# Corleone-Huang/DynamicVectorQuantization

Hardware: AMD Instinct MI355X
Metric: images encoded/sec (VQ hot path: gate + routing + VQ assign), 256x256 inputs, K=1024 (higher is better)
Workload: dtype f32; 1 GPU; BASELINE configs[2]: dqvae-entropy-dual-r05, B=256 per GPU, 32x32x256 latents, K=1024, entropy gate + dual routing + VectorQuantize2 assign as one op (quant_conv not in the path); global_batch=256, assign_mode=filter, spinup_steps=100, streams=3, repeats=1, full=False, parallelism=single GPU: no exchange runs, world=1, distinct_devices=1

## Files before the change

dynamicvectorquantization_amd/csrc/dvq_pass1.h:

```cpp
#pragma once
#include "dvq_filter.h"
#include <type_traits>

#define DVQ_LOAD_Z(p) __builtin_nontemporal_load(p)
#define DVQ_STORE_ZQ(p, v) __builtin_nontemporal_store((v), (p))
#define DVQ_BUF_LOAD(rsrc, voff, soff, AUX) __builtin_bit_cast(float, __builtin_amdgcn_raw_buffer_load_b32((rsrc), (voff), (soff), (AUX)))
#define DVQ_BUF_STORE(v, rsrc, voff, soff) __builtin_amdgcn_raw_buffer_store_b32(__builtin_bit_cast(unsigned, (float)(v)), (rsrc), (voff), (soff), 2)
#define DVQ_BUF_LOAD16(XT, rsrc, voff, soff, AUX) dvq_widen_bits<XT>(__builtin_amdgcn_raw_buffer_load_b16((rsrc), (voff), (soff), (AUX)))
#define DVQ_BUF_STORE16(XT, v, rsrc, voff, soff) __builtin_amdgcn_raw_buffer_store_b16(dvq_narrow_bits<XT>(v), (rsrc), (voff), (soff), 2)
#define DVQ_LOAD_SEL(p) (*(p))

#ifdef DVQ_TUNING
#ifdef __HIP_DEVICE_COMPILE__
#define DVQ_TUNING_PTR __device__
#else
#define DVQ_TUNING_PTR static __device__
#endif
DVQ_TUNING_PTR float *g_dvq_tokdbg __asm__("g_dvq_tokdbg") = nullptr;
DVQ_TUNING_PTR unsigned long long *g_dvq_stamps __asm__("g_dvq_stamps") = nullptr;
#define DVQ_STAMP(i) do { if (SPLIT && g_dvq_stamps != nullptr && threadIdx.x == 0) g_dvq_stamps[(size_t)blockIdx.x * 8 + (i)] = wall_clock64(); } while (0)
static inline int dvq_tuning_set_unit(void *stamps, void *tokdbg)
{
    int rc = (int)hipMemcpyToSymbol(HIP_SYMBOL(g_dvq_stamps), &stamps, sizeof(void *));
    if (rc) return rc;
// ... 78 lines not shown
        if constexpr (RES) {
#pragma unroll
            for (int k = 0; k < SEED_TILES / 2 / NW; ++k) {
                const int pair = wave * (SEED_TILES / 2 / NW) + k;
                const int t0 = (2 * pair < T) ? 2 * pair : T - 1;
                const unsigned voff = (unsigned)c * 4u + ((t0 + 1 < T) ? (unsigned)h * (unsigned)TILE_STRIDE : 0u);
                glds4(img + (size_t)t0 * TILE_STRIDE + IMG_BYTES + voff, enraw + pair * 64);
            }
        }
    };
    const int tile_id = SPLIT ? (int)(blockIdx.x / (unsigned)ksplit) : xcd_swizzle(blockIdx.x, gridDim.x);
    const int pre = (SEL == 2) ? ((rv.G == 2) ? 2 : 1) : 3;

    const int n_raw = (tile_id * NW + wave) * 32 + c;
    const int n = (n_raw < N) ? n_raw : -1;
    auto token_base = [&](int HW, int h) -> size_t {
        const long nn = (n >= 0) ? n : N - 1;
        if constexpr (FLAT) return (size_t)nn * D + 8 * h;
        const long bimg = nn / HW;
        const int hw = (int)(nn - bimg * HW);
        return ((size_t)bimg * D + 8 * h) * HW + hw;
    };
    auto wave_base = [&](const float *p0, int hw, int hh) -> __amdgpu_buffer_rsrc_t {
        const size_t tb = token_base(hw, hh);
        const size_t tb0 = ((size_t)(unsigned)__builtin_amdgcn_readfirstlane((int)(tb >> 32)) << 32) |
                           (size_t)(unsigned)__builtin_amdgcn_readfirstlane((int)(tb & 0xFFFFFFFFu));
        if constexpr (XT != 0) return __builtin_amdgcn_make_buffer_rsrc((void *)((const char *)p0 + tb0 * ZB), 0, -1, 0x00020000);
        else return __builtin_amdgcn_make_buffer_rsrc((void *)(p0 + tb0), 0, -1, 0x00020000);
    };
    auto lane_off = [&](int hw, int hh) -> unsigned {
        const size_t tb = token_base(hw, hh);
        const size_t tb0 = ((size_t)(unsigned)__builtin_amdgcn_readfirstlane((int)(tb >> 32)) << 32) |
                           (size_t)(unsigned)__builtin_amdgcn_readfirstlane((int)(tb & 0xFFFFFFFFu));
        return (unsigned)(tb - tb0) * (XT ? 2u : 4u);
    };
    float zf[S16][8];
    float sel_mask = 1.0f;
    int sel_g = 0;
    unsigned stg_a = 0, stg_b = 0;
    auto conv_prologue = [&](const float *zp, size_t st) __attribute__((always_inline)) {
        constexpr int QIMG = S16 * 1024;
        constexpr int QTILE = 2 * QIMG + 256;
        float *bias_l = enraw;
        float xr[3][8];
        const float *xp = zp;
        auto issue_w = [&](int k, int q) __attribute__((always_inline)) {
            const int i = 4 * wave + q;
            glds16(cv.wimg + (size_t)(i >> 1) * QTILE + (i & 1) * QIMG + k * 1024 + lane * 16,
                   lds + (k & 3) * IMG_BYTES + i * 1024);
        };
        auto issue_x = [&](int k, int j) __attribute__((always_inline)) {
            asm volatile("global_load_dword %0, %1, off nt" : "=v"(xr[k % 3][j]) : "v"(xp) : "memory");
            xp += (j == 7) ? 9 * st : st;
        };
        auto issue_group = [&](int k) __attribute__((always_inline)) {
#pragma unroll
            for (int q = 0; q < 4; ++q) issue_w(k, q);
#pragma unroll
            for (int j = 0; j < 8; ++j) issue_x(k, j);
        };
        glds4(cv.bias + wave * 64 + lane, bias_l + wave * 64);
        issue_group(0);
        issue_group(1);
        issue_group(2);
        f32x16 acc[8];
#pragma unroll
        for (int t8 = 0; t8 < 8; ++t8)
#pragma unroll
            for (int r = 0; r < 16; ++r) acc[t8][r] = 0.0f;
        int ea = 100;
        float sa = ldexpf(1.0f, 100);
        f16x8 xh, xl;
        auto take_group = [&](int g) __attribute__((always_inline)) {
            if (g <= S16 - 3) asm volatile("s_waitcnt vmcnt(24)" ::: "memory");
            else if (g == S16 - 2) asm volatile("s_waitcnt vmcnt(12)" ::: "memory");
            else asm volatile("s_waitcnt vmcnt(0)" ::: "memory");
            float xv[8];
#pragma unroll
            for (int j = 0; j < 8; ++j) { asm volatile("" : "+v"(xr[g % 3][j])); xv[j] = xr[g % 3][j]; }
            float m = 0.0f;
#pragma unroll
            for (int j = 0; j < 8; ++j) m = vmax_abs(m, xv[j]);
            m = fmaxf(m, __shfl_xor(m, 32));
            const bool grow = (m > 0.0f) && (m < __builtin_inff()) && (m * sa >= 32768.0f);
            if (__builtin_amdgcn_ballot_w64(grow) != 0ull) {
                int e;
                (void)frexpf(grow ? m : 1.0f, &e);
                int en = 14 - e;
                en = en > 100 ? 100 : (en < -100 ? -100 : en);
                en = grow ? en : ea;
                if (g > 0) {
                    const float f = ldexpf(1.0f, en - ea);
#pragma unroll
                    for (int t8 = 0; t8 < 8; ++t8)
#pragma unroll
                        for (int r = 0; r < 16; ++r) acc[t8][r] *= f;
                }
                ea = en;
                sa = ldexpf(1.0f, ea);
            }
            u32x4 ph, pl;
#pragma unroll
            for (int j2 = 0; j2 < 4; ++j2) {
                const float v0 = xv[2 * j2] * sa, v1 = xv[2 * j2 + 1] * sa;
                const f32x2 vv = {v0, v1};
                const f16x2 hh = __builtin_convertvector(vv, f16x2);
                const f32x2 rr = {v0 - (float)hh[0], v1 - (float)hh[1]};
                const f16x2 ll = __builtin_convertvector(rr, f16x2);
                ph[j2] = __builtin_bit_cast(unsigned, hh);
                pl[j2] = __builtin_bit_cast(unsigned, ll);
            }
            xh = __builtin_bit_cast(f16x8, ph);
            xl = __builtin_bit_cast(f16x8, pl);
        };
        take_group(0);
#pragma unroll
        for (int s = 0; s < S16; ++s) {
            __builtin_amdgcn_s_barrier();
            asm volatile("" ::: "memory");
            const f16x8 bh = xh, bl = xl;
            const unsigned wa = (unsigned)(size_t)(const __attribute__((address_space(3))) char *)(lds + (s & 3) * IMG_BYTES) + lane * 16;
            f16x8 wf[3];
#define CV_OFF(Q) ((((Q) & 1) ? ((Q) - 1) : ((Q) + 1)) * 1024)
#define CV_RD(Q) asm volatile("ds_read_b128 %0, %1 offset:%c2" : "=v"(wf[(Q) % 3]) : "v"(wa), "i"(CV_OFF(Q)))
#define CV_WAIT(N, Q) asm volatile("s_waitcnt lgkmcnt(" #N ")" : "+v"(wf[(Q) % 3]) :: "memory")
            CV_RD(0); CV_RD(1); CV_RD(2);
            __builtin_amdgcn_sched_barrier(0);
#define CV_TILE(T8, W0, W1)                                                                                              \
            CV_WAIT(W0, 2 * (T8));                                                                                        \
            __builtin_amdgcn_sched_barrier(0);                                                                            \
            acc[T8] = __builtin_amdgcn_mfma_f32_32x32x16_f16(wf[(2 * (T8)) % 3], bh, acc[T8], 0, 0, 0);    \
            __builtin_amdgcn_sched_barrier(0);                                                                            \
            if (2 * (T8) + 3 < 16) { CV_RD(2 * (T8) + 3 < 16 ? 2 * (T8) + 3 : 0); }                                       \
            CV_WAIT(W1, 2 * (T8) + 1);                                                                                    \
            __builtin_amdgcn_sched_barrier(0);                                                                            \
            acc[T8] = __builtin_amdgcn_mfma_f32_32x32x16_f16(wf[(2 * (T8) + 1) % 3], bl, acc[T8], 0, 0, 0);               \
            acc[T8] = __builtin_amdgcn_mfma_f32_32x32x16_f16(wf[(2 * (T8) + 1) % 3], bh, acc[T8], 0, 0, 0);               \
            __builtin_amdgcn_sched_barrier(0);                                                                            \
            if (2 * (T8) + 4 < 16) { CV_RD(2 * (T8) + 4 < 16 ? 2 * (T8) + 4 : 0); }
#define CV_W(Q) if (s + 3 < S16) { issue_w(s + 3, Q); __builtin_amdgcn_sched_barrier(0); }
#define CV_X(J) if (s + 3 < S16) { issue_x(s + 3, J); issue_x(s + 3, (J) + 1); __builtin_amdgcn_sched_barrier(0); }
            CV_TILE(0, 2, 2) CV_W(0) CV_TILE(1, 2, 2) CV_W(1) CV_TILE(2, 2, 2) CV_W(2) CV_TILE(3, 2, 2) CV_W(3)
            CV_TILE(4, 2, 2) CV_X(0) CV_TILE(5, 2, 2) CV_X(2) CV_TILE(6, 2, 2) CV_X(4) CV_TILE(7, 1, 0) CV_X(6)
#undef CV_W
#undef CV_X
#undef CV_TILE
#undef CV_WAIT
#undef CV_RD
#undef CV_OFF
            __builtin_amdgcn_sched_barrier(0);
            if (s + 1 < S16) take_group(s + 1);
        }
        const float unscale = ldexpf(cv.meta->inv_scale_w, -ea);
#pragma unroll
        for (int s = 0; s < S16; ++s) {
            const f32x4 b0 = *(const f32x4 *)(bias_l + 16 * s + 8 * h), b1v = *(const f32x4 *)(bias_l + 16 * s + 8 * h + 4);
#pragma unroll
            for (int j = 0; j < 8; ++j)
                zf[s][j] = __builtin_fmaf(acc[s >> 1][8 * (s & 1) + j], unscale, (j < 4) ? b0[j & 3] : b1v[j & 3]);
            __builtin_amdgcn_sched_barrier(0);
        }
        if (cv.h_all && n >= 0) {
            float *hp = cv.h_buf + token_base(HW, h);
#pragma unroll
            for (int s = 0; s < S16; ++s)
#pragma unroll
                for (int j = 0; j < 8; ++j) hp[(size_t)(16 * s + j) * HW] = zf[s][j];
        }
        __builtin_amdgcn_s_barrier();
        asm volatile("" ::: "memory");
        issue_seeds();
        for (int t = 0; t < 3; ++t) issue(t);
        __builtin_amdgcn_sched_barrier(0);
    };
    if (SEL != 0) {
        const int nn = (n >= 0) ? n : (int)(N - 1);
        const int b = nn / HW, pos = nn - b * HW;
        const int y = pos / rv.Wout, x = pos - y * rv.Wout;
        const int SC = rv.sub[rv.G - 1];
        const size_t cell = (size_t)b * rv.hc * rv.wc + (y / SC) * rv.wc + x / SC;
        const DvqGateRaw graw = dvq_gate_fetch(rv.gate, rv.gate_mode, rv.G, cell);
        auto by_products = [&](int g) {
            const int rep_g = rv.rep[g];
            sel_mask = 1.0f / (float)(rep_g * rep_g);
            if (n >= 0 && h == 0 && rv.cmask_out != nullptr) {
                rv.cmask_out[n] = sel_mask;
                if (y % SC == 0 && x % SC == 0) {
                    rv.indices_out[cell] = g;
                    if (rv.gate_mode == 2 && rv.gate_out != nullptr) {
                        const float e = graw.f[0];
                        longlong2 gg; gg.x = (e <= rv.thr) ? 1 : 0; gg.y = (e > rv.thr) ? 1 : 0;
                        *(longlong2 *)(rv.gate_out + 2 * cell) = gg;
                    }
                }
            }
            if (!(y % rep_g == 0 && x % rep_g == 0)) sel_mask = -sel_mask;
        };
        if (SEL == 1) {
            const int g = dvq_gate_reduce(graw, rv.gate_mode, rv.G, rv.thr);
            by_products(g);
            int stride_l;
            const float *zp = dvq_dense_source(rv, b, y, x, g, stride_l) + (size_t)8 * h * stride_l;
            const size_t st = (size_t)stride_l;
            if constexpr (CONV) {
                conv_prologue(zp, st);
            } else {
            issue_seeds();
            for (int t = 0; t < pre; ++t) issue(t);
            __builtin_amdgcn_s_setprio(2);
#pragma unroll
            for (int s = 0; s < S16; ++s)
#pragma unroll
                for (int j = 0; j < 8; ++j) zf[s][j] = DVQ_LOAD_SEL(zp + (size_t)(16 * s + j) * st);
            __builtin_amdgcn_s_setprio(0);
            }
        } else {
            issue_seeds();
            for (int t = 0; t < pre; ++t) issue(t);
            const int bw = __builtin_amdgcn_readfirstlane(b);
            const int y0 = __builtin_amdgcn_readfirstlane(y) - wave;
            char *img_a = lds + pre * IMG_BYTES;
            char *img_b = lds + 3 * IMG_BYTES;
            {
                const int ga = rv.G - 2;
                const int plane = rv.hc * rv.sub[ga] * 16;
                const float *src = rv.src[ga] + (size_t)bw * D * plane + (size_t)(y0 >> 1) * 16 + (lane & 7) * 4;
                for (int i = wave; i < D / 8; i += NW)
                    glds16(src + (size_t)(i * 8 + (lane >> 3)) * plane, img_a + i * 1024);
            }
            if (rv.G == 3) {
                const int plane = rv.hc * 8;
                const float *src = rv.src[0] + (size_t)bw * D * plane + (size_t)(y0 >> 2) * 8 + (lane & 1) * 4;
                for (int i = wave; i < D / 32; i += NW)
                    glds16(src + (size_t)(i * 32 + (lane >> 1)) * plane, img_b + i * 1024);
            }
            stg_a = (unsigned)(size_t)(const __attribute__((address_space(3))) char *)img_a +
                    (unsigned)((8 * h) * 128 + (((wave >> 1) * 16 + (c >> 1)) << 2));
            stg_b = (unsigned)(size_t)(const __attribute__((address_space(3))) char *)img_b +
                    (unsigned)((8 * h) * 32 + ((c >> 2) << 2));
            const __amdgpu_buffer_rsrc_t zr = __builtin_amdgcn_make_buffer_rsrc((void *)(rv.src[rv.G - 1] + (size_t)bw * D * HW), 0,
                                                                                -1, 0x00020000);
            const unsigned zo = (unsigned)(8 * h * HW + pos) * 4u;
            __builtin_amdgcn_s_setprio(2);
#pragma unroll
            for (int s = 0; s < S16; ++s)
#pragma unroll
                for (int j = 0; j < 8; ++j) zf[s][j] = DVQ_BUF_LOAD(zr, zo, (16 * s + j) * HW * 4, NT ? 2 : 0);
            __builtin_amdgcn_s_setprio(0);
            asm volatile("s_waitcnt vmcnt(0)" ::: "memory");
            __builtin_amdgcn_s_barrier();
            asm volatile("" ::: "memory");
            sel_g = dvq_gate_reduce(graw, rv.gate_mode, rv.G, rv.thr);
            by_products(sel_g);
        }
    } else if constexpr (CONV) {
        conv_prologue(z + token_base(HW, h), (size_t)HW);
    } else if constexpr (FLAT) {
        char *tr = lds + wave * FLAT_TRW;
        const long n0 = ((long)tile_id * NW + wave) * 32;
        f32x4 tmp[2][FLAT_IPH];
#pragma unroll
        for (int h2 = 0; h2 < 2; ++h2)
#pragma unroll
            for (int i = 0; i < FLAT_IPH; ++i) {
                long tk = n0 + i * FLAT_TPI + lane / FLAT_LPT;
                tk = tk < N ? tk : N - 1;
                const f32x4 *src = (const f32x4 *)(z + (size_t)tk * D + h2 * (D / 2)) + (lane % FLAT_LPT);
                tmp[h2][i] = NT ? __builtin_nontemporal_load(src) : *src;
            }
#pragma unroll
        for (int h2 = 0; h2 < 2; ++h2) {
#pragma unroll
            for (int i = 0; i < FLAT_IPH; ++i)
                *(f32x4 *)(tr + (i * FLAT_TPI + lane / FLAT_LPT) * FLAT_RSH + (lane % FLAT_LPT) * 16) = tmp[h2][i];
#pragma unroll
            for (int sp = 0; sp < S16 / 2; ++sp) {
                const int s = h2 * (S16 / 2) + sp;
                const f32x4 lo = *(const f32x4 *)(tr + c * FLAT_RSH + (16 * sp + 8 * h) * 4);
                const f32x4 hi = *(const f32x4 *)(tr + c * FLAT_RSH + (16 * sp + 8 * h + 4) * 4);
#pragma unroll
                for (int j = 0; j < 4; ++j) { zf[s][j] = lo[j]; zf[s][4 + j] = hi[j]; }
            }
        }
        __syncthreads();
        issue_seeds();
        for (int t = 0; t < pre; ++t) issue(t);
    } else {
        issue_seeds();
        for (int t = 0; t < pre; ++t) issue(t);
        const __amdgpu_buffer_rsrc_t zr = wave_base(z, HW, h);
        const unsigned zo = lane_off(HW, h);
        __builtin_amdgcn_s_setprio(2);
#pragma unroll
        for (int s = 0; s < S16; ++s)
#pragma unroll
            for (int j = 0; j < 8; ++j) {
                if constexpr (XT != 0) zf[s][j] = DVQ_BUF_LOAD16(XT, zr, zo, (16 * s + j) * HW * 2, NT ? 2 : 0);
                else zf[s][j] = DVQ_BUF_LOAD(zr, zo, (16 * s + j) * HW * 4, NT ? 2 : 0);
            }
        __builtin_amdgcn_s_setprio(0);
    }
    f16x8 zb[2][S32];
    float xn, thr2W;
    {
        float pa[2][8];
        float amax = 0.0f, zeta2 = 0.0f;
        f16x8 zprev = {};
#pragma unroll
        for (int s = 0; s < S16; ++s) {
            if (SEL == 2) {
                if (sel_g == rv.G - 2) {
#pragma unroll
                    for (int j = 0; j < 8; ++j)
                        asm volatile("ds_read_b32 %0, %1 offset:%c2" : "+v"(zf[s][j]) : "v"(stg_a), "i"((16 * s + j) * 128));
                    asm volatile("s_waitcnt lgkmcnt(0)" ::: "memory");
                }
                if (rv.G == 3 && sel_g == 0) {
#pragma unroll
                    for (int j = 0; j < 8; ++j)
                        asm volatile("ds_read_b32 %0, %1 offset:%c2" : "+v"(zf[s][j]) : "v"(stg_b), "i"((16 * s + j) * 32));
                    asm volatile("s_waitcnt lgkmcnt(0)" ::: "memory");
                }
#pragma unroll
                for (int j = 0; j < 8; ++j) asm volatile("" : "+v"(zf[s][j]));
            }
            u32x4 packed;
#pragma unroll
            for (int j2 = 0; j2 < 4; ++j2) {
                const float v0 = zf[s][2 * j2], v1 = zf[s][2 * j2 + 1];
                const float q0 = sq_rn(v0), q1 = sq_rn(v1);
                pa[s & 1][2 * j2] = (s < 2) ? q0 : __fadd_rn(pa[s & 1][2 * j2], q0);
                pa[s & 1][2 * j2 + 1] = (s < 2) ? q1 : __fadd_rn(pa[s & 1][2 * j2 + 1], q1);
                amax = vmax_abs(amax, v0);
                amax = vmax_abs(amax, v1);
                f32x2 vv = {v0, v1};
                f16x2 hh = __builtin_convertvector(vv, f16x2);
                packed[j2] = __builtin_bit_cast(unsigned, hh);
                const float r0 = v0 - (float)hh[0], r1 = v1 - (float)hh[1];
                zeta2 = __builtin_fmaf(r0, r0, zeta2);
                zeta2 = __builtin_fmaf(r1, r1, zeta2);
            }
            if constexpr (SEL == 2) {
                asm volatile("" : "+v"(packed), "+v"(zeta2));
                if (sel_mask < 0.0f) packed = u32x4{0u, 0u, 0u, 0u};
            }
            const f16x8 zcur = __builtin_bit_cast(f16x8, packed);
            if (s & 1) {
                const int sp = s >> 1;
                *(f16x8 *)(scr + lane * 16) = zprev;
                *(f16x8 *)(scr + 1024 + lane * 16) = zcur;
#pragma unroll
                for (int t2 = 0; t2 < 2; ++t2) {
                    const int srcl = 16 * t2 + (lane & 15) + 32 * ((lane >> 4) & 1);
                    zb[t2][sp] = *(const f16x8 *)(scr + (lane >> 5) * 1024 + srcl * 16);
                }
            }
            zprev = zcur;
            if constexpr (CONV) __builtin_amdgcn_sched_barrier(0);
        }
        float t8[8];
#pragma unroll
        for (int l = 0; l < 8; ++l) {
            float o0 = __shfl_xor(pa[0][l], 32), o1 = __shfl_xor(pa[1][l], 32);
            float a0 = h == 0 ? pa[0][l] : o0;
            float a1 = h == 0 ? o0 : pa[0][l];
            float a2 = h == 0 ? pa[1][l] : o1;
            float a3 = h == 0 ? o1 : pa[1][l];
            t8[l] = __fadd_rn(__fadd_rn(__fadd_rn(a0, a1), a2), a3);
        }
        xn = t8[0];
#pragma unroll
        for (int l = 1; l < 8; ++l) xn = __fadd_rn(xn, t8[l]);
        amax = fmaxf(amax, __shfl_xor(amax, 32));
        zeta2 += __shfl_xor(zeta2, 32);
        thr2W = FOLD ? dvq_fold_threshold(xn, amax, zeta2, sB, (const DvqFoldMeta *)meta)
                     : dvq_filter_threshold(xn, amax, zeta2, sB, meta);
    }
    if (SEL == 2) {
        __builtin_amdgcn_s_barrier();
        asm volatile("" ::: "memory");
    }
    for (int t = pre; t < 3; ++t) issue(t);
    DVQ_STAMP(1);

    float best, second;
    int code;
    {
        const int q16 = lane >> 4;
        float b1[2] = {-__builtin_inff(), -__builtin_inff()}, b2[2] = {-__builtin_inff(), -__builtin_inff()};
        int bt[2] = {0, 0};
        f32x4 acc16[2][2];
        auto top2 = [&](int tt) {
#pragma unroll
            for (int t2 = 0; t2 < 2; ++t2) {
                const float om = b1[t2];
#pragma unroll
                for (int r = 0; r < 8; r += 2) {
                    const float v0 = acc16[r >> 2][t2][r & 3], v1 = acc16[(r + 1) >> 2][t2][(r + 1) & 3];
                    float g0 = __uint_as_float((__float_as_uint(v0) & 0xFFFFFFF0u) | (unsigned)r);
                    float g1 = __uint_as_float((__float_as_uint(v1) & 0xFFFFFFF0u) | (unsigned)(r + 1));
                    float md = __builtin_amdgcn_fmed3f(b1[t2], g0, g1);
                    b1[t2] = vmax3_raw(b1[t2], g0, g1);
                    b2[t2] = vmax_raw(b2[t2], md);
                }
                bt[t2] = (b1[t2] != om) ? tt : bt[t2];
            }
        };
    for (int t = 0; t < T; ++t) {
            asm volatile("s_waitcnt vmcnt(%0)" ::"n"(PER_TILE) : "memory");
            __builtin_amdgcn_s_barrier();
            asm volatile("" ::: "memory");
            if (S16 != 16) issue(t + 3);
            const unsigned tile_a = (unsigned)(size_t)(const __attribute__((address_space(3))) char *)(
                                        lds + (t & (NBUF - 1)) * IMG_BYTES + lane * 16);
            f16x8 a0, a1, a2, a3;
#define DVQ_RD(dst, S) asm volatile("ds_read_b128 %0, %1 offset:%c2" : "=v"(dst) : "v"(tile_a), "i"((S) * 1024))
            DVQ_RD(a0, 0); DVQ_RD(a1, 1); DVQ_RD(a2, 2); DVQ_RD(a3, 3);
            __builtin_amdgcn_sched_barrier(0);
            if (t > 0) top2(t - 1);
            __builtin_amdgcn_sched_barrier(0);
            {
                const unsigned seed_a = (unsigned)(size_t)(const __attribute__((address_space(3))) char *)(
                                            RES ? enraw + t * 32 + 4 * q16 : enraw + ((t & (NBUF - 1)) * NW + wave) * 64 + 4 * q16);
                f32x4 e0, e1;
                asm volatile("ds_read_b128 %0, %1" : "=v"(e0) : "v"(seed_a));
                asm volatile("ds_read_b128 %0, %1 offset:64" : "=v"(e1) : "v"(seed_a));
                asm volatile("s_waitcnt lgkmcnt(0)" : "+v"(e0), "+v"(e1), "+v"(a0), "+v"(a1), "+v"(a2), "+v"(a3) :: "memory");
                acc16[0][0] = e0; acc16[0][1] = e0; acc16[1][0] = e1; acc16[1][1] = e1;
            }
            __builtin_amdgcn_sched_barrier(0);
#define DVQ_PIECE(Q) if constexpr ((Q) < PER_TILE) { issue_piece(t + 3, Q); }
#define DVQ_MM(src, F, WAIT, NEXT)                                                                             \
            asm volatile("s_waitcnt lgkmcnt(" #WAIT ")" ::: "memory");                                            \
            __builtin_amdgcn_sched_barrier(0);                                                                    \
            acc16[(F) / S32][0] = __builtin_amdgcn_mfma_f32_16x16x32_f16(src, zb[0][(F) % S32], acc16[(F) / S32][0], 0, 0, 0); \
            acc16[(F) / S32][1] = __builtin_amdgcn_mfma_f32_16x16x32_f16(src, zb[1][(F) % S32], acc16[(F) / S32][1], 0, 0, 0); \
            __builtin_amdgcn_sched_barrier(0);                                                                    \
            if ((F) + 4 < S16) { DVQ_RD(src, ((F) + 4 < S16 ? (F) + 4 : 0)); }                                  \
            NEXT
            __builtin_amdgcn_s_setprio(1);
            if (S16 == 16) {
                DVQ_MM(a0, 0, 0, ) DVQ_MM(a1, 1, 1, DVQ_PIECE(0)) DVQ_MM(a2, 2, 2, ) DVQ_MM(a3, 3, 3, )
                DVQ_MM(a0, 4, 3, DVQ_PIECE(1)) DVQ_MM(a1, 5, 3, ) DVQ_MM(a2, 6, 3, ) DVQ_MM(a3, 7, 3, DVQ_PIECE(2))
                DVQ_MM(a0, 8, 3, ) DVQ_MM(a1, 9, 3, ) DVQ_MM(a2, 10, 3, DVQ_PIECE(3)) DVQ_MM(a3, 11, 3, )
                DVQ_MM(a0, 12, 3, ) DVQ_MM(a1, 13, 2, DVQ_PIECE(4)) DVQ_MM(a2, 14, 1, ) DVQ_MM(a3, 15, 0, )
            } else if (S16 == 8) {
                DVQ_MM(a0, 0, 0, ) DVQ_MM(a1, 1, 1, ) DVQ_MM(a2, 2, 2, ) DVQ_MM(a3, 3, 3, )
                DVQ_MM(a0, 4, 3, ) DVQ_MM(a1, 5, 2, ) DVQ_MM(a2, 6, 1, ) DVQ_MM(a3, 7, 0, )
            } else {
                DVQ_MM(a0, 0, 0, ) DVQ_MM(a1, 1, 0, ) DVQ_MM(a2, 2, 0, ) DVQ_MM(a3, 3, 0, )
            }
#undef DVQ_MM
#undef DVQ_RD
#undef DVQ_PIECE
            __builtin_amdgcn_s_setprio(0);
        }
        top2(T - 1);
        asm volatile("s_waitcnt vmcnt(0)" ::: "memory");
        float rb[2], rs[2];
        int rc[2];
#pragma unroll
        for (int t2 = 0; t2 < 2; ++t2) {
            float mb = b1[t2], ms = b2[t2];
            int mt = bt[t2], mq = q16;
#pragma unroll
            for (int off = 16; off <= 32; off <<= 1) {
                const float o1 = __shfl_xor(mb, off), o2 = __shfl_xor(ms, off);
                const int ot = __shfl_xor(mt, off), oq = __shfl_xor(mq, off);
                const bool other_wins = (o1 > mb) || (o1 == mb && ((lane ^ off) < lane));
                ms = fmaxf(other_wins ? mb : o1, fmaxf(ms, o2));
                mb = other_wins ? o1 : mb;
                mt = other_wins ? ot : mt;
                mq = other_wins ? oq : mq;
            }
            const int r = (int)(__float_as_uint(mb) & 15u);
            rb[t2] = mb;
            rs[t2] = ms;
            rc[t2] = (mt + t_lo) * 32 + 16 * (r >> 2) + 4 * mq + (r & 3);
        }
        const int srcl = c & 15;
        const float x0 = __shfl(rb[0], srcl), x1 = __shfl(rb[1], srcl);
        const float y0 = __shfl(rs[0], srcl), y1 = __shfl(rs[1], srcl);
        const int c0 = __shfl(rc[0], srcl), c1 = __shfl(rc[1], srcl);
        best = (c >> 4) ? x1 : x0;
        second = (c >> 4) ? y1 : y0;
        code = (c >> 4) ? c1 : c0;
    }
    DVQ_STAMP(2);
    if constexpr (SEL == 2) {
        const int lane_e = (int)__builtin_amdgcn_mbcnt_hi(~0u, __builtin_amdgcn_mbcnt_lo(~0u, 0u));
        const int c_e = lane_e & 31;
        float am = __builtin_fabsf(sel_mask);
        asm volatile("" : "+v"(am));
        const int rm1 = (am == 1.0f) ? 0 : ((am == 0.25f) ? 1 : 3);
        char *hand = lds + NBUF * IMG_BYTES + NBUF * NW * 64 * 4;
        if (lane_e < 32) {
            const f32x4 mine = {best, second, __int_as_float(code), 0.0f};
            *(f32x4 *)(hand + wave * 2048 + c_e * 16) = mine;
        }
        __syncthreads();
        const f32x4 own = *(const f32x4 *)(hand + (wave - (wave & rm1)) * 2048 + (c_e - (c_e & rm1)) * 16);
        best = own[0];
        second = own[1];
        code = __float_as_int(own[2]);
    }
    if constexpr (SPLIT) {
        typedef __attribute__((address_space(1))) unsigned long long gu64;
        __shared__ int s_last;
        gu64 *mine = (gu64 *)(split + ((size_t)tile_id * ksplit) * 128 + wave * 32 + c);
        if (h == 0) {
            gu64 *e = mine + (size_t)ks * 128 * 2;
            __hip_atomic_store(e, ((unsigned long long)__float_as_uint(second) << 32) | __float_as_uint(best), __ATOMIC_RELAXED, __HIP_MEMORY_SCOPE_AGENT);
            __hip_atomic_store(e + 1, (unsigned long long)(unsigned)code, __ATOMIC_RELAXED, __HIP_MEMORY_SCOPE_AGENT);
        }
        asm volatile("s_waitcnt vmcnt(0)" ::: "memory");
        __syncthreads();
        DVQ_STAMP(3);
        if (tid == 0) {
            const int old = __hip_atomic_fetch_add(&counters[DVQ_SPLIT_TICKET0 + tile_id], 1, __ATOMIC_RELAXED, __HIP_MEMORY_SCOPE_AGENT);
            s_last = (old == ksplit - 1);
            if (old == ksplit - 1)
                __hip_atomic_store(&counters[DVQ_SPLIT_TICKET0 + tile_id], 0, __ATOMIC_RELAXED, __HIP_MEMORY_SCOPE_AGENT);
        }
        __syncthreads();
        DVQ_STAMP(4);
        if (!s_last) return;
        float mb = -__builtin_inff(), ms = -__builtin_inff();
        int mc = 0;
        unsigned long long e0[DVQ_SPLIT_MAX_SLICES], e1[DVQ_SPLIT_MAX_SLICES];
#pragma unroll
        for (int k = 0; k < DVQ_SPLIT_MAX_SLICES; ++k) {
            const int kk = k < ksplit ? k : ksplit - 1;
            e0[k] = __hip_atomic_load(mine + (size_t)kk * 128 * 2, __ATOMIC_RELAXED, __HIP_MEMORY_SCOPE_AGENT);
            e1[k] = __hip_atomic_load(mine + (size_t)kk * 128 * 2 + 1, __ATOMIC_RELAXED, __HIP_MEMORY_SCOPE_AGENT);
        }
#pragma unroll
        for (int k = 0; k < DVQ_SPLIT_MAX_SLICES; ++k) {
            const float eb = __uint_as_float((unsigned)e0[k]), es = __uint_as_float((unsigned)(e0[k] >> 32));
            const bool other_wins = k < ksplit && eb > mb;
            ms = (k < ksplit) ? fmaxf(other_wins ? mb : eb, fmaxf(ms, es)) : ms;
            mc = other_wins ? (int)(unsigned)e1[k] : mc;
            mb = other_wins ? eb : mb;
        }
        best = mb; second = ms; code = mc;
        DVQ_STAMP(5);
    }
    const float thr = best - thr2W;
    const bool final_ok = (best - second) > thr2W;
    const bool valid = n >= 0;
    bool hopeless = !(code < K) || !(thr == thr);
#ifdef DVQ_TUNING
    if (g_dvq_tokdbg != nullptr && valid && h == 0) {
        f32x4 dbg = {best, second, thr2W, (float)code};
        *(f32x4 *)(g_dvq_tokdbg + 4 * (size_t)n) = dbg;
    }
#endif
    const bool undecided = valid && !hopeless && !final_ok;
    const int sel_rep = (SEL == 0 || sel_mask < 0.0f) ? (SEL == 0 ? 1 : 0) : (sel_mask == 1.0f ? 1 : (sel_mask == 0.25f ? 2 : 4));
    const bool queued = undecided && sel_rep > 0;
    const unsigned long long umask = __ballot(queued && h == 0);
    const int shard = (SPLIT ? tile_id * NW + wave : (int)blockIdx.x) & (DVQ_QSHARDS - 1);
    int slot_raw = 0;
    if (umask != 0ull && lane == 0) slot_raw = atomicAdd(&counters[DVQ_QCOUNT0 + shard], (int)__popcll(umask));
    if (valid && hopeless && h == 0) {
        int pos = atomicAdd(&counters[DVQ_C_EXACT], 1);
        exact_list[pos] = n;
    }
    float lsum = 0.0f;
    float m_tok = 1.0f;
    if (valid && !hopeless) {
        if (h == 0) codes[n] = (long long)code;
        m_tok = (SEL != 0) ? __builtin_fabsf(sel_mask) : ((mask != nullptr) ? mask[n] : 1.0f);
        if (zq != nullptr || partials != nullptr) {
            int h_e = h;
            if constexpr (FOLD || (FLAT && SPLIT) || SEL == 2) h_e =(int)(__builtin_amdgcn_mbcnt_hi(~0u, __builtin_amdgcn_mbcnt_lo(~0u, 0u)) >> 5);
            const float *ep = E + (size_t)code * D + 8 * h_e;
            constexpr int SB = SPLIT ? ((S16 < 8) ? S16 : 8) : ((S16 < 2) ? S16 : 2);
            auto finish = [&](auto store_tag) {
                constexpr bool STORE = decltype(store_tag)::value;
                int hw_e = HW;
                asm volatile("" : "+s"(hw_e));
                const __amdgpu_buffer_rsrc_t qr = wave_base(STORE ? zq : (float *)E, hw_e, h_e);
                const unsigned qo = lane_off(hw_e, h_e);
                int hw4 = HW * (XT ? 2 : 4);
                asm volatile("" : "+s"(hw4));
#pragma unroll
                for (int s0 = 0; s0 < S16; s0 += SB) {
                    f32x4 eg[SB][2];
#pragma unroll
                    for (int q = 0; q < SB; ++q) {
                        eg[q][0] = *(const f32x4 *)(ep + 16 * (s0 + q));
                        eg[q][1] = *(const f32x4 *)(ep + 16 * (s0 + q) + 4);
                    }
#pragma unroll
                    for (int q = 0; q < SB; ++q) {
                        const int s = s0 + q;
#pragma unroll
                        for (int j = 0; j < 8; ++j) {
                            float e = eg[q][j >> 2][j & 3];
                            if constexpr (FOLD) {
                                if (STORE) DVQ_BUF_STORE(e, qr, qo, (16 * s + j) * hw4);
                            } else {
                            float diff = __fsub_rn(e, zf[s][j]);
                            if constexpr (XT != 0) {
                                if (STORE) DVQ_BUF_STORE16(XT, __fadd_rn(zf[s][j], diff), qr, qo, (16 * s + j) * hw4);
                            } else
                            if (STORE) DVQ_BUF_STORE(__fadd_rn(zf[s][j], diff), qr, qo, (16 * s + j) * hw4);
                            lsum = __builtin_fmaf(diff, diff, lsum);
                            }
                        }
                    }
                }
            };
            if constexpr (!FLAT) {
                if (zq != nullptr) finish(std::true_type{});
                else finish(std::false_type{});
                lsum *= m_tok;
            }
        }
    }
    if constexpr (FLAT) {
        char *flat_tr = lds + wave * FLAT_TRW;
        const bool store = zq != nullptr;
        if (store) __syncthreads();
        const bool mine = valid && !hopeless && (store || partials != nullptr);
        const unsigned long long okmask = __ballot(valid && !hopeless && h == 0);
        const long n0 = ((long)tile_id * NW + wave) * 32;
        const float *ep = E + (size_t)(mine ? code : 0) * D + 8 * h;
#pragma unroll
        for (int h2 = 0; h2 < 2; ++h2) {
            if (mine) {
                constexpr int SB = (S16 / 2 < 2) ? S16 / 2 : 2;
#pragma unroll
                for (int sp0 = 0; sp0 < S16 / 2; sp0 += SB) {
                    f32x4 eg[SB][2];
#pragma unroll
                    for (int q = 0; q < SB; ++q) {
                        eg[q][0] = *(const f32x4 *)(ep + 16 * (h2 * (S16 / 2) + sp0 + q));
                        eg[q][1] = *(const f32x4 *)(ep + 16 * (h2 * (S16 / 2) + sp0 + q) + 4);
                    }
#pragma unroll
                    for (int q = 0; q < SB; ++q) {
                        const int sp = sp0 + q, s = h2 * (S16 / 2) + sp;
                        f32x4 o[2];
#pragma unroll
                        for (int j = 0; j < 8; ++j) {
                            const float e = eg[q][j >> 2][j & 3];
                            if constexpr (FOLD) {
                                o[j >> 2][j & 3] = e;
                            } else {
                                const float diff = __fsub_rn(e, zf[s][j]);
                                o[j >> 2][j & 3] = __fadd_rn(zf[s][j], diff);
                                lsum = __builtin_fmaf(diff, diff, lsum);
                            }
                        }
                        if (store) {
                            *(f32x4 *)(flat_tr + c * FLAT_RSH + (16 * sp + 8 * h) * 4) = o[0];
                            *(f32x4 *)(flat_tr + c * FLAT_RSH + (16 * sp + 8 * h + 4) * 4) = o[1];
                        }
                    }
                }
            }
            if (store) {
#pragma unroll
                for (int i = 0; i < FLAT_IPH; ++i) {
                    const int tk = i * FLAT_TPI + lane / FLAT_LPT;
                    const f32x4 v = *(const f32x4 *)(flat_tr + tk * FLAT_RSH + (lane % FLAT_LPT) * 16);
                    if ((okmask >> tk) & 1ull)
                        __builtin_nontemporal_store(v, (f32x4 *)(zq + (size_t)(n0 + tk) * D + h2 * (D / 2)) + (lane % FLAT_LPT));
                }
            }
        }
        lsum *= m_tok;
    }
    DVQ_STAMP(6);
    if (umask != 0ull) {
        const int base = __shfl(slot_raw, 0);
        int slot = base + (int)__popcll(umask & ((1ull << c) - 1ull));
        slot = queued ? slot : -1;
        if (queued && slot >= rec_cap) {
            if (h == 0) {
                const int rr = sel_rep > 0 ? sel_rep : 1;
                for (int ry = 0; ry < rr; ++ry)
                    for (int rx = 0; rx < rr; ++rx) {
                        int pos = atomicAdd(&counters[DVQ_C_EXACT], 1);
                        exact_list[pos] = n + ry * rv.Wout + rx;
                    }
            }
            lsum = -(float)(sel_rep * sel_rep - 1) * lsum;
            slot = -1;
        }
        if (slot >= 0) {
            char *rec = records + ((size_t)shard * rec_cap + slot) * rec_bytes(D);
#pragma unroll
            for (int s = 0; s < S16; ++s) {
                f32x4 lo = {zf[s][0], zf[s][1], zf[s][2], zf[s][3]};
                f32x4 hi = {zf[s][4], zf[s][5], zf[s][6], zf[s][7]};
                *(f32x4 *)(rec + (16 * s + 8 * h) * 4) = lo;
                *(f32x4 *)(rec + (16 * s + 8 * h + 4) * 4) = hi;
            }
            if (h == 0) {
                RecMeta rm;
                rm.n = n; rm.xn = xn; rm.thr = thr; rm.m = m_tok; rm.prov = code;
                rm.best = ~0ull; rm.rep = sel_rep > 0 ? sel_rep : 1;
                *(RecMeta *)(rec + (size_t)D * 4) = rm;
            }
        }
    }
    if (partials != nullptr) {
        double dsum = (double)lsum;
#pragma unroll
        for (int off = 32; off > 0; off >>= 1) dsum += __shfl_xor(dsum, off);
        __syncthreads();
        double *red = (double *)lds;
        if (lane == 0) red[wave] = dsum;
        __syncthreads();
        if (tid == 0) partials[SPLIT ? tile_id : (int)blockIdx.x] = (red[0] + red[1]) + (red[2] + red[3]);
    }
    DVQ_STAMP(7);
}

template <int D, int SEL, bool CONV, bool FOLD, bool RES>
__global__ __launch_bounds__(256, 2) void vq_assign_filter_kernel(
    const float *__restrict__ z, const char *__restrict__ img, const DvqF16Meta *__restrict__ meta,
    const float *__restrict__ E, const float *__restrict__ mask,
    int HW, int K, long N, float *__restrict__ zq, long long *__restrict__ codes,
    double *__restrict__ partials, int *__restrict__ counters, int *__restrict__ exact_list,
    char *__restrict__ records, int rec_cap, const DvqRouted rv, const DvqConv cv)
{
    pass1_body<D, SEL, CONV, FOLD, true, RES>(z, img, meta, E, mask, HW, K, N, zq, codes, partials, counters, exact_list, records, rec_cap, rv, cv);
}

template <int D, bool FOLD, bool RES>
__global__ __launch_bounds__(256, 2) void vq_assign_filter_flat_kernel(
    const float *__restrict__ z, const char *__restrict__ img, const DvqF16Meta *__restrict__ meta,
    const float *__restrict__ E, const float *__restrict__ mask,
    int HW, int K, long N, float *__restrict__ zq, long long *__restrict__ codes,
    double *__restrict__ partials, int *__restrict__ counters, int *__restrict__ exact_list,
    char *__restrict__ records, int rec_cap, const DvqRouted rv, const DvqConv cv)
{
    pass1_body<D, 0, false, FOLD, true, RES, true>(z, img, meta, E, mask, HW, K, N, zq, codes, partials, counters, exact_list, records, rec_cap, rv, cv);
}

template <int D, int SEL, bool CONV, bool FOLD, bool FLAT, bool RES>
__global__ __launch_bounds__(256, 2) void vq_assign_filter_split_kernel(
    const float *__restrict__ z, const char *__restrict__ img, const DvqF16Meta *__restrict__ meta,
    const float *__restrict__ E, const float *__restrict__ mask,
    int HW, int K, long N, float *__restrict__ zq, long long *__restrict__ codes,
    double *__restrict__ partials, int *__restrict__ counters, int *__restrict__ exact_list,
    char *__restrict__ records, int rec_cap, const DvqRouted rv, const DvqConv cv, f32x4 *__restrict__ split, int ksplit)
{
    pass1_body<D, SEL, CONV, FOLD, CONV, RES, FLAT, true>(z, img, meta, E, mask, HW, K, N, zq, codes, partials, counters, exact_list, records,
                                                     rec_cap, rv, cv, split, ksplit);
}

template <int D, int SEL, bool FOLD, bool RES>
__global__ __launch_bounds__(256, 2) void vq_assign_filter_cached_kernel(
    const float *__restrict__ z, const char *__restrict__ img, const DvqF16Meta *__restrict__ meta,
    const float *__restrict__ E, const float *__restrict__ mask,
    int HW, int K, long N, float *__restrict__ zq, long long *__restrict__ codes,
    double *__restrict__ partials, int *__restrict__ counters, int *__restrict__ exact_list,
    char *__restrict__ records, int rec_cap, const DvqRouted rv, const DvqConv cv)
{
    pass1_body<D, SEL, false, FOLD, false, RES>(z, img, meta, E, mask, HW, K, N, zq, codes, partials, counters, exact_list, records, rec_cap, rv, cv);
}

template <int D, bool RES, int XT>
__global__ __launch_bounds__(256, 2) void vq_assign_filter_x16_kernel(
    const void *__restrict__ z, const char *__restrict__ img, const DvqF16Meta *__restrict__ meta,
    const float *__restrict__ E, const float *__restrict__ mask,
    int HW, int K, long N, void *__restrict__ zq, long long *__restrict__ codes,
    double *__restrict__ partials, int *__restrict__ counters, int *__restrict__ exact_list,
    char *__restrict__ records, int rec_cap)
{
    static_assert(XT == 1 || XT == 2, "f16 or bf16");
    pass1_body<D, 0, false, false, true, RES, false, false, XT>((const float *)z, img, meta, E, mask, HW, K, N, (float *)zq, codes, partials,
                                                                counters, exact_list, records, rec_cap, DvqRouted{}, DvqConv{});
}

struct FilterWs {
    int *counters, *chunk_sync, *exact_list;
    char *records;
    int cap;
    f32x4 *split;
};

enum class P1Form { plain, cached, flat, split, wide, x16 };
struct P1Plan {
    P1Form form;
// ... 121 lines not shown
```

Baseline: 1.324 million images/s.

## Compact live token columns and skip half the MFMAs when enough are masked

For the dual-routing select path, builds a per-wave permutation that packs active token columns first and masked copy columns last, so the B operand layout places live tokens in the first 16-column group. When at least 16 columns are masked copies, a single-group variant of the distance loop runs, issuing half the MFMAs and top-2 updates. Results are then un-permuted with a popcount-based lane map. This adds an LDS table, extra ballot/popcount logic and a duplicated, wave-uniform-branched loop body that increases code size and register pressure.

```diff
diff --git a/dynamicvectorquantization_amd/csrc/dvq_pass1.h b/dynamicvectorquantization_amd/csrc/dvq_pass1.h
--- a/dynamicvectorquantization_amd/csrc/dvq_pass1.h
+++ b/dynamicvectorquantization_amd/csrc/dvq_pass1.h
@@ -404,6 +404,20 @@
     }
     f16x8 zb[2][S32];
     float xn, thr2W;
+    unsigned copymask = 0u;
+    unsigned perm_off[2] = {0u, 0u};
+    if constexpr (SEL == 2) {
+        copymask = (unsigned)__builtin_amdgcn_ballot_w64(sel_mask < 0.0f && h == 0);
+        const int below = __builtin_popcount(copymask & ((1u << c) - 1u));
+        const int p = (sel_mask < 0.0f) ? 32 - __builtin_popcount(copymask) + below : c - below;
+        unsigned char *tab = (unsigned char *)scr;
+        if (h == 0) tab[p] = (unsigned char)c;
+#pragma unroll
+        for (int t2 = 0; t2 < 2; ++t2) {
+            const unsigned col = tab[16 * t2 + (lane & 15)];
+            perm_off[t2] = (unsigned)(lane >> 5) * 1024u + (col + 32u * ((unsigned)(lane >> 4) & 1u)) * 16u;
+        }
+    }
     {
         float pa[2][8];
         float amax = 0.0f, zeta2 = 0.0f;
@@ -453,8 +467,12 @@
                 *(f16x8 *)(scr + 1024 + lane * 16) = zcur;
 #pragma unroll
                 for (int t2 = 0; t2 < 2; ++t2) {
+                    if constexpr (SEL == 2) {
+                        zb[t2][sp] = *(const f16x8 *)(scr + perm_off[t2]);
+                    } else {
                     const int srcl = 16 * t2 + (lane & 15) + 32 * ((lane >> 4) & 1);
                     zb[t2][sp] = *(const f16x8 *)(scr + (lane >> 5) * 1024 + srcl * 16);
+                    }
                 }
             }
             zprev = zcur;
@@ -491,73 +509,21 @@
         const int q16 = lane >> 4;
         float b1[2] = {-__builtin_inff(), -__builtin_inff()}, b2[2] = {-__builtin_inff(), -__builtin_inff()};
         int bt[2] = {0, 0};
-        f32x4 acc16[2][2];
-        auto top2 = [&](int tt) {
-#pragma unroll
-            for (int t2 = 0; t2 < 2; ++t2) {
-                const float om = b1[t2];
-#pragma unroll
-                for (int r = 0; r < 8; r += 2) {
-                    const float v0 = acc16[r >> 2][t2][r & 3], v1 = acc16[(r + 1) >> 2][t2][(r + 1) & 3];
-                    float g0 = __uint_as_float((__float_as_uint(v0) & 0xFFFFFFF0u) | (unsigned)r);
-                    float g1 = __uint_as_float((__float_as_uint(v1) & 0xFFFFFFF0u) | (unsigned)(r + 1));
-                    float md = __builtin_amdgcn_fmed3f(b1[t2], g0, g1);
-                    b1[t2] = vmax3_raw(b1[t2], g0, g1);
-                    b2[t2] = vmax_raw(b2[t2], md);
-                }
-                bt[t2] = (b1[t2] != om) ? tt : bt[t2];
-            }
-        };
-    for (int t = 0; t < T; ++t) {
-            asm volatile("s_waitcnt vmcnt(%0)" ::"n"(PER_TILE) : "memory");
-            __builtin_amdgcn_s_barrier();
-            asm volatile("" ::: "memory");
-            if (S16 != 16) issue(t + 3);
-            const unsigned tile_a = (unsigned)(size_t)(const __attribute__((address_space(3))) char *)(
-                                        lds + (t & (NBUF - 1)) * IMG_BYTES + lane * 16);
-            f16x8 a0, a1, a2, a3;
-#define DVQ_RD(dst, S) asm volatile("ds_read_b128 %0, %1 offset:%c2" : "=v"(dst) : "v"(tile_a), "i"((S) * 1024))
-            DVQ_RD(a0, 0); DVQ_RD(a1, 1); DVQ_RD(a2, 2); DVQ_RD(a3, 3);
-            __builtin_amdgcn_sched_barrier(0);
-            if (t > 0) top2(t - 1);
-            __builtin_amdgcn_sched_barrier(0);
-            {
-                const unsigned seed_a = (unsigned)(size_t)(const __attribute__((address_space(3))) char *)(
-                                            RES ? enraw + t * 32 + 4 * q16 : enraw + ((t & (NBUF - 1)) * NW + wave) * 64 + 4 * q16);
-                f32x4 e0, e1;
-                asm volatile("ds_read_b128 %0, %1" : "=v"(e0) : "v"(seed_a));
-                asm volatile("ds_read_b128 %0, %1 offset:64" : "=v"(e1) : "v"(seed_a));
-                asm volatile("s_waitcnt lgkmcnt(0)" : "+v"(e0), "+v"(e1), "+v"(a0), "+v"(a1), "+v"(a2), "+v"(a3) :: "memory");
-                acc16[0][0] = e0; acc16[0][1] = e0; acc16[1][0] = e1; acc16[1][1] = e1;
-            }
-            __builtin_amdgcn_sched_barrier(0);
-#define DVQ_PIECE(Q) if constexpr ((Q) < PER_TILE) { issue_piece(t + 3, Q); }
-#define DVQ_MM(src, F, WAIT, NEXT)                                                                             \
-            asm volatile("s_waitcnt lgkmcnt(" #WAIT ")" ::: "memory");                                            \
-            __builtin_amdgcn_sched_barrier(0);                                                                    \
-            acc16[(F) / S32][0] = __builtin_amdgcn_mfma_f32_16x16x32_f16(src, zb[0][(F) % S32], acc16[(F) / S32][0], 0, 0, 0); \
-            acc16[(F) / S32][1] = __builtin_amdgcn_mfma_f32_16x16x32_f16(src, zb[1][(F) % S32], acc16[(F) / S32][1], 0, 0, 0); \
-            __builtin_amdgcn_sched_barrier(0);                                                                    \
-            if ((F) + 4 < S16) { DVQ_RD(src, ((F) + 4 < S16 ? (F) + 4 : 0)); }                                  \
-            NEXT
-            __builtin_amdgcn_s_setprio(1);
-            if (S16 == 16) {
-                DVQ_MM(a0, 0, 0, ) DVQ_MM(a1, 1, 1, DVQ_PIECE(0)) DVQ_MM(a2, 2, 2, ) DVQ_MM(a3, 3, 3, )
-                DVQ_MM(a0, 4, 3, DVQ_PIECE(1)) DVQ_MM(a1, 5, 3, ) DVQ_MM(a2, 6, 3, ) DVQ_MM(a3, 7, 3, DVQ_PIECE(2))
-                DVQ_MM(a0, 8, 3, ) DVQ_MM(a1, 9, 3, ) DVQ_MM(a2, 10, 3, DVQ_PIECE(3)) DVQ_MM(a3, 11, 3, )
-                DVQ_MM(a0, 12, 3, ) DVQ_MM(a1, 13, 2, DVQ_PIECE(4)) DVQ_MM(a2, 14, 1, ) DVQ_MM(a3, 15, 0, )
-            } else if (S16 == 8) {
-                DVQ_MM(a0, 0, 0, ) DVQ_MM(a1, 1, 1, ) DVQ_MM(a2, 2, 2, ) DVQ_MM(a3, 3, 3, )
-                DVQ_MM(a0, 4, 3, ) DVQ_MM(a1, 5, 2, ) DVQ_MM(a2, 6, 1, ) DVQ_MM(a3, 7, 0, )
+        if constexpr (SEL == 2) {
+            if (__builtin_popcount(copymask) >= 16) {
+#define DVQ_NG 1
+#include "pass1_loop.h"
+#undef DVQ_NG
             } else {
-                DVQ_MM(a0, 0, 0, ) DVQ_MM(a1, 1, 0, ) DVQ_MM(a2, 2, 0, ) DVQ_MM(a3, 3, 0, )
-            }
-#undef DVQ_MM
-#undef DVQ_RD
-#undef DVQ_PIECE
-            __builtin_amdgcn_s_setprio(0);
-        }
-        top2(T - 1);
+#define DVQ_NG 2
+#include "pass1_loop.h"
+#undef DVQ_NG
+            }
+        } else {
+#define DVQ_NG 2
+#include "pass1_loop.h"
+#undef DVQ_NG
+        }
         asm volatile("s_waitcnt vmcnt(0)" ::: "memory");
         float rb[2], rs[2];
         int rc[2];
@@ -580,6 +546,20 @@
             rs[t2] = ms;
             rc[t2] = (mt + t_lo) * 32 + 16 * (r >> 2) + 4 * mq + (r & 3);
         }
+        if constexpr (SEL == 2) {
+            unsigned cm = copymask;
+            asm volatile("" : "+s"(cm));
+            const int c_p = (int)__builtin_amdgcn_mbcnt_hi(~0u, __builtin_amdgcn_mbcnt_lo(~0u, 0u)) & 31;
+            const int below = __builtin_popcount(cm & ((1u << c_p) - 1u));
+            const int pc = ((cm >> c_p) & 1u) ? 32 - __builtin_popcount(cm) + below : c_p - below;
+            const int srcl = pc & 15;
+            const float x0 = __shfl(rb[0], srcl), x1 = __shfl(rb[1], srcl);
+            const float y0 = __shfl(rs[0], srcl), y1 = __shfl(rs[1], srcl);
+            const int c0 = __shfl(rc[0], srcl), c1 = __shfl(rc[1], srcl);
+            best = (pc >> 4) ? x1 : x0;
+            second = (pc >> 4) ? y1 : y0;
+            code = (pc >> 4) ? c1 : c0;
+        } else {
         const int srcl = c & 15;
         const float x0 = __shfl(rb[0], srcl), x1 = __shfl(rb[1], srcl);
         const float y0 = __shfl(rs[0], srcl), y1 = __shfl(rs[1], srcl);
@@ -587,6 +567,7 @@
         best = (c >> 4) ? x1 : x0;
         second = (c >> 4) ? y1 : y0;
         code = (c >> 4) ? c1 : c0;
+        }
     }
     DVQ_STAMP(2);
     if constexpr (SEL == 2) {
diff --git a/dynamicvectorquantization_amd/csrc/pass1_loop.h b/dynamicvectorquantization_amd/csrc/pass1_loop.h
--- /dev/null
+++ b/dynamicvectorquantization_amd/csrc/pass1_loop.h
@@ -0,0 +1,69 @@
+        f32x4 acc16[2][2];
+        auto top2 = [&](int tt) {
+#pragma unroll
+            for (int t2 = 0; t2 < DVQ_NG; ++t2) {
+                const float om = b1[t2];
+#pragma unroll
+                for (int r = 0; r < 8; r += 2) {
+                    const float v0 = acc16[r >> 2][t2][r & 3], v1 = acc16[(r + 1) >> 2][t2][(r + 1) & 3];
+                    float g0 = __uint_as_float((__float_as_uint(v0) & 0xFFFFFFF0u) | (unsigned)r);
+                    float g1 = __uint_as_float((__float_as_uint(v1) & 0xFFFFFFF0u) | (unsigned)(r + 1));
+                    float md = __builtin_amdgcn_fmed3f(b1[t2], g0, g1);
+                    b1[t2] = vmax3_raw(b1[t2], g0, g1);
+                    b2[t2] = vmax_raw(b2[t2], md);
+                }
+                bt[t2] = (b1[t2] != om) ? tt : bt[t2];
+            }
+        };
+    for (int t = 0; t < T; ++t) {
+            asm volatile("s_waitcnt vmcnt(%0)" ::"n"(PER_TILE) : "memory");
+            __builtin_amdgcn_s_barrier();
+            asm volatile("" ::: "memory");
+            if (S16 != 16) issue(t + 3);
+            const unsigned tile_a = (unsigned)(size_t)(const __attribute__((address_space(3))) char *)(
+                                        lds + (t & (NBUF - 1)) * IMG_BYTES + lane * 16);
+            f16x8 a0, a1, a2, a3;
+#define DVQ_RD(dst, S) asm volatile("ds_read_b128 %0, %1 offset:%c2" : "=v"(dst) : "v"(tile_a), "i"((S) * 1024))
+            DVQ_RD(a0, 0); DVQ_RD(a1, 1); DVQ_RD(a2, 2); DVQ_RD(a3, 3);
+            __builtin_amdgcn_sched_barrier(0);
+            if (t > 0) top2(t - 1);
+            __builtin_amdgcn_sched_barrier(0);
+            {
+                const unsigned seed_a = (unsigned)(size_t)(const __attribute__((address_space(3))) char *)(
+                                            RES ? enraw + t * 32 + 4 * q16 : enraw + ((t & (NBUF - 1)) * NW + wave) * 64 + 4 * q16);
+                f32x4 e0, e1;
+                asm volatile("ds_read_b128 %0, %1" : "=v"(e0) : "v"(seed_a));
+                asm volatile("ds_read_b128 %0, %1 offset:64" : "=v"(e1) : "v"(seed_a));
+                asm volatile("s_waitcnt lgkmcnt(0)" : "+v"(e0), "+v"(e1), "+v"(a0), "+v"(a1), "+v"(a2), "+v"(a3) :: "memory");
+                acc16[0][0] = e0; if (DVQ_NG == 2) acc16[0][1] = e0;
+                acc16[1][0] = e1; if (DVQ_NG == 2) acc16[1][1] = e1;
+            }
+            __builtin_amdgcn_sched_barrier(0);
+#define DVQ_PIECE(Q) if constexpr ((Q) < PER_TILE) { issue_piece(t + 3, Q); }
+#define DVQ_MM(src, F, WAIT, NEXT)                                                                             \
+            asm volatile("s_waitcnt lgkmcnt(" #WAIT ")" ::: "memory");                                            \
+            __builtin_amdgcn_sched_barrier(0);                                                                    \
+            acc16[(F) / S32][0] = __builtin_amdgcn_mfma_f32_16x16x32_f16(src, zb[0][(F) % S32], acc16[(F) / S32][0], 0, 0, 0); \
+            if (DVQ_NG == 2)                                                                                      \
+            acc16[(F) / S32][1] = __builtin_amdgcn_mfma_f32_16x16x32_f16(src, zb[1][(F) % S32], acc16[(F) / S32][1], 0, 0, 0); \
+            __builtin_amdgcn_sched_barrier(0);                                                                    \
+            if ((F) + 4 < S16) { DVQ_RD(src, ((F) + 4 < S16 ? (F) + 4 : 0)); }                                  \
+            NEXT
+            __builtin_amdgcn_s_setprio(1);
+            if (S16 == 16) {
+                DVQ_MM(a0, 0, 0, ) DVQ_MM(a1, 1, 1, DVQ_PIECE(0)) DVQ_MM(a2, 2, 2, ) DVQ_MM(a3, 3, 3, )
+                DVQ_MM(a0, 4, 3, DVQ_PIECE(1)) DVQ_MM(a1, 5, 3, ) DVQ_MM(a2, 6, 3, ) DVQ_MM(a3, 7, 3, DVQ_PIECE(2))
+                DVQ_MM(a0, 8, 3, ) DVQ_MM(a1, 9, 3, ) DVQ_MM(a2, 10, 3, DVQ_PIECE(3)) DVQ_MM(a3, 11, 3, )
+                DVQ_MM(a0, 12, 3, ) DVQ_MM(a1, 13, 2, DVQ_PIECE(4)) DVQ_MM(a2, 14, 1, ) DVQ_MM(a3, 15, 0, )
+            } else if (S16 == 8) {
+                DVQ_MM(a0, 0, 0, ) DVQ_MM(a1, 1, 1, ) DVQ_MM(a2, 2, 2, ) DVQ_MM(a3, 3, 3, )
+                DVQ_MM(a0, 4, 3, ) DVQ_MM(a1, 5, 2, ) DVQ_MM(a2, 6, 1, ) DVQ_MM(a3, 7, 0, )
+            } else {
+                DVQ_MM(a0, 0, 0, ) DVQ_MM(a1, 1, 0, ) DVQ_MM(a2, 2, 0, ) DVQ_MM(a3, 3, 0, )
+            }
+#undef DVQ_MM
+#undef DVQ_RD
+#undef DVQ_PIECE
+            __builtin_amdgcn_s_setprio(0);
+        }
+        top2(T - 1);
```

After: 1.357 million images/s, median of 6. 1.02x the previous value.
